# esteinig/sketchy

Hardware: AMD Instinct MI355X
Metric: reads/sec streamed (s=10000,k=16,40k-genome ref) (higher is better)
Workload: dtype u64

## Files before the change

### sketchy_amd/csrc/skx_capi.hip

```cpp
#include <dlfcn.h>
#include <hip/hip_runtime.h>
#include <rccl/rccl.h>

#include <unistd.h>

#include <algorithm>
#include <atomic>
#include <chrono>
#include <cmath>
#include <condition_variable>
#include <cstdarg>
#include <cstdio>
#include <cstdlib>
#include <cstring>
#include <mutex>
#include <string>
#include <thread>
#include <unordered_map>
#include <vector>

#include "sketchy_hip.h"
#include "skx_common.hpp"
#include "skx_genome_groups.hpp"
#include "skx_kernels.hpp"
// ... 965 lines not shown
    u32* h_nq_sink = nullptr;
    u32* h_nd = nullptr;
    u32 *d_rowcnt = nullptr;
    skx::SlotExtents rowcnt_ext;
    bool front_open = false;
    void extents_unknown() { rowcnt_ext.whole(); for (auto& q : ps) { q.smap_ext.whole(); q.mqc_whole = 0xFFu; } }
    u32 *d_gain = nullptr;
    u32 *d_gain_s = nullptr;
    u32 *d_candslot = nullptr;
    u32 *d_candmask = nullptr;
    uint2 *d_lrow = nullptr;
    u32 *d_nlrow = nullptr, *d_gain_l = nullptr, *d_cbase = nullptr, *d_cwl = nullptr, *d_ncwl = nullptr;
    u64 *d_cw = nullptr;
    u64 *d_inb = nullptr, *d_hit = nullptr;
    skx::LongRows long_rows() const { return skx::LongRows{d_lrow, d_nlrow, qcap + 128, d_inb, ref->n_lw}; }
    bool use_pat = false;
    u32 *d_hist = nullptr, *d_nprow = nullptr;
    u64* d_pcw = nullptr;
    u32 npat_pad = 0;
    skx::PatRows pat_rows() const { return skx::PatRows{d_hist, npat_pad, d_gain_l, d_nprow}; }
    skx::RareIndex rare_index() const {
        skx::RareIndex ri = ref->rare_index();
        if (!use_pat) { ri.prec = nullptr; ri.n_pat = 0; }
        if (!static_dense) { ri.qs = nullptr; ri.n_sd = 0; }
        return ri;
    }
    u32 *d_cbad = nullptr, *d_nqc = nullptr;
    u32 *d_spc_g0 = nullptr, *d_spc_grp = nullptr;
    u32 n_pad_c = 0, n_grp_c = 0, cand_seq = 0;
    struct PassSet {
// ... 185 lines not shown
    if (!st) return;
    (void)hipSetDevice(st->device);
    if (st->hs0) (void)hipStreamSynchronize(st->hs0);
    if (st->hs1) (void)hipStreamSynchronize(st->hs1);
    if (st->hs) (void)hipStreamSynchronize(st->hs);
    if (st->hs2) (void)hipStreamSynchronize(st->hs2);
    for (int i = 1; i < skx_stream::kRankLanes; ++i)
        if (st->lane[i].s) (void)hipStreamSynchronize(st->lane[i].s);
    for (int i = 0; i < kSides; ++i) (void)hipFree(st->sd_rows[i]);
    void* ptrs[] = {st->d_bases, st->d_offsets, st->d_pair_h[0], st->d_pair_h[1],
                    st->d_q[0], st->d_q[1], st->d_pair_r[0], st->d_pair_r[1], st->d_pair_q[0], st->d_pair_q[1],
                    st->d_poff_pass[0], st->d_poff_pass[1], st->d_poff_pass[2], st->d_pair_r[2], st->d_nq[0], st->d_nq[1], st->d_win[0], st->d_win[1], st->d_m, st->d_mint, st->d_mq[0], st->d_mq[1],
                    st->d_topk_idx, st->d_topk_sum, st->d_cons, st->d_ev.n_events, st->d_ev.ev_read, st->d_ev.ev_idx, st->d_ev.ev_sum, st->d_ev.ev_codes, st->d_tab_tmp, st->d_rank_idx, st->d_rank_sum, st->d_bsum, st->d_grp_any[0],
                    st->d_grp_any[1], st->d_hbuf, st->d_wb[0], st->d_wb[1], st->d_rowany[0], st->d_rowany[1], st->d_mqext,
                    st->d_qd, st->d_qrow, st->d_sslot, st->d_qinfo, st->d_qloc, st->d_cls_bsum, st->d_nd_hs,
                    st->d_rowcnt, st->d_gain, st->d_gain_s, st->d_candslot, st->d_candmask, st->d_lrow, st->d_nlrow, st->d_gain_l, st->d_cbase, st->d_cwl, st->d_ncwl, st->d_cw, st->d_cbad, st->d_nqc, st->d_spc_g0, st->d_spc_grp, st->d_inb, st->d_hit, st->d_hist, st->d_nprow, st->d_pcw, st->d_ms[0], st->d_ms[1], st->d_mdirty_s};
    for (auto& q : st->ps) {
        for (void* x : {(void*)q.tab, (void*)q.cand, (void*)q.tabc, (void*)q.ncand, (void*)q.mode, (void*)q.any_full, (void*)q.nqc_total, (void*)q.mc, (void*)q.mqc,
                        (void*)q.rowany_c, (void*)q.grp_any_c, (void*)q.smap, (void*)q.pair_qc, (void*)q.nd}) (void)hipFree(x);
        if (q.h_pub) (void)hipHostFree(q.h_pub);
    }
    for (auto& t : st->d_tab) (void)hipFree(t);
    for (int i = 0; i < skx_stream::kRankLanes; ++i) free_lane(st, i);
    for (int i = 1; i < skx_stream::kRankLanes; ++i)
        if (st->own_lane_stream && st->lane[i].s) (void)hipStreamDestroy(st->lane[i].s);
    for (void* p : ptrs) (void)hipFree(p);
    stats_free(st->stats);
    if (st->h_poff) (void)hipHostFree(st->h_poff);
    if (st->h_offsets) (void)hipHostFree(st->h_offsets);
    if (st->h_nq) (void)hipHostFree(st->h_nq);
    if (st->h_nd) (void)hipHostFree(st->h_nd);
// ... 433 lines not shown
            SCHK(hipMalloc(&st->d_cbase, (size_t)nb * (n_pad / 64) * 4));
            SCHK(hipMalloc(&st->d_cwl, (size_t)nb * st->n_pad_c * 4));
            SCHK(hipMalloc(&st->d_ncwl, 64));
            if (ref->d_mlongT) {
                SCHK(hipMalloc(&st->d_inb, (size_t)nb * ref->n_lw * 8));
                SCHK(hipMalloc(&st->d_hit, (size_t)nb * ref->n_lw * 8));
            }
            if (ref->d_prec && ref->n_pat && st->n_grp_c * skx::kRankWords <= skx::pat_words_max()) {
                st->use_pat = true;
                st->npat_pad = (ref->n_pat + 63u) & ~63u;
                SCHK(hipMalloc(&st->d_hist, (size_t)nb * st->npat_pad * 4));
                SCHK(hipMalloc(&st->d_nprow, skx::pass_counter_bytes()));
                SCHK(hipMalloc(&st->d_pcw, (size_t)nb * ref->n_pat * st->n_grp_c * skx::kRankWords * 8));
            }
        }
        SCHK(hipMalloc(&st->d_cbad, 64));
        SCHK(hipMalloc(&st->d_nqc, skx::pass_counter_bytes()));
        std::vector<u32> g0c(n_sp), grpc(st->n_grp_c);
        for (u32 i = 0; i < n_sp; ++i) g0c[i] = i * cap;
        for (u32 i = 0; i < st->n_grp_c; ++i) grpc[i] = i / (cap / (skx::kRankWords * 64));
        SCHK(hipMalloc(&st->d_spc_g0, (size_t)n_sp * 4));
        SCHK(hipMalloc(&st->d_spc_grp, (size_t)st->n_grp_c * 4));
        SCHK(hipMemcpy(st->d_spc_g0, g0c.data(), (size_t)n_sp * 4, hipMemcpyHostToDevice));
        SCHK(hipMemcpy(st->d_spc_grp, grpc.data(), (size_t)st->n_grp_c * 4, hipMemcpyHostToDevice));
        for (auto& q : st->ps) {
            SCHK(hipMalloc(&q.tab, (size_t)(nb + 1) * n_pad * 8));
            SCHK(hipMalloc(&q.cand, (size_t)nb * st->n_pad_c * 4));
            SCHK(hipMalloc(&q.tabc, (size_t)nb * st->n_pad_c * 8));
            SCHK(hipMalloc(&q.ncand, (size_t)nb * n_sp * 4));
            SCHK(hipMalloc(&q.mode, 64)); SCHK(hipMalloc(&q.any_full, 64)); SCHK(hipMalloc(&q.nqc_total, 64));
// ... 103 lines not shown
    const size_t mq_words = (size_t)((n_gw + skx::kRankWords - 1) / skx::kRankWords * skx::kRankWords);
    for (hipStream_t h : {st->hs0, st->hs1, st->hs, st->hs2}) if (h) HIPCHK(hipStreamSynchronize(h));
    for (int i = 1; i < st->n_lanes; ++i) if (st->lane[i].s) HIPCHK(hipStreamSynchronize(st->lane[i].s));
    size_t mem_free = 0, mem_total = 0;
    HIPCHK(hipMemGetInfo(&mem_free, &mem_total));
    const u64 per_row = (st->static_dense ? 0 : (u64)n_pad / 8 * (st->d_mint ? 2 : 1)) + 2 * mq_words * 8 + 2 * (u64)(n_pad / (skx::kRankWords * 64)) / 8 + 1 +
                        5ull * skx::kPassBatchesMax * 4;
    want_rows += st->sd64;
    static const int grow_div = skx::knob("SKX_GROW_DIV") ? std::max(1, atoi(skx::knob("SKX_GROW_DIV"))) : 4;
    u64 rows = std::min<u64>(want_rows, (u64)(mem_free / grow_div) / per_row);
    rows = std::min<u64>(rows, st->pcap) / 64 * 64;
    if (rows <= st->qcap) return SKX_OK;
    u64 *m = nullptr, *mint = nullptr, *mq[2] = {nullptr, nullptr}, *ra[2] = {nullptr, nullptr};
    u32 *wb[2] = {nullptr, nullptr}, *cnt = nullptr, *sm[2] = {nullptr, nullptr};
    uint2* lrow = nullptr;
    auto undo = [&]() { for (void* q : {(void*)m, (void*)mint, (void*)mq[0], (void*)mq[1], (void*)ra[0], (void*)ra[1], (void*)wb[0], (void*)wb[1], (void*)cnt, (void*)sm[0], (void*)sm[1], (void*)lrow}) if (q) (void)hipFree(q); (void)hipGetLastError(); };
    hipError_t e = st->static_dense ? hipSuccess : hipMalloc(&m, (size_t)(rows / 64 + 2) * n_pad * 8);
    if (e == hipSuccess && st->d_mint) e = hipMalloc(&mint, (size_t)(rows / 64 + 2) * n_pad * 8);
    for (int i = 0; i < 2 && e == hipSuccess; ++i) e = hipMalloc(&mq[i], ((size_t)rows + 128) * mq_words * 8);
    for (int i = 0; i < 2 && e == hipSuccess; ++i) e = hipMalloc(&ra[i], (size_t)(n_pad / (skx::kRankWords * 64)) * (rows / 64 + 2) * 8);
    for (int i = 0; i < 2 && e == hipSuccess && st->d_wb[i]; ++i) e = hipMalloc(&wb[i], ((size_t)rows / 64 + 1) * ref->n_tiles * 16);
    if (e == hipSuccess) e = hipMalloc(&cnt, (size_t)skx::kPassBatchesMax * ((size_t)rows + 128) * 4);
    if (e == hipSuccess && st->d_lrow) e = hipMalloc(&lrow, (size_t)skx::kPassBatchesMax * ((size_t)rows + 128) * 8);
    for (int i = 0; i < 2 && e == hipSuccess; ++i) e = hipMalloc(&sm[i], (size_t)skx::kPassBatchesMax * ((size_t)rows + 128) * 4);
    if (e == hipSuccess && m) e = hipMemset(m, 0, (size_t)(rows / 64 + 2) * n_pad * 8);
    for (int i = 0; i < 2 && e == hipSuccess; ++i) e = hipMemset(mq[i], 0, ((size_t)rows + 128) * mq_words * 8);
    for (int i = 0; i < 2 && e == hipSuccess; ++i) e = hipMemset(ra[i], 0, (size_t)(n_pad / (skx::kRankWords * 64)) * (rows / 64 + 2) * 8);
    if (e == hipSuccess) {
        const u32 any[4] = {skx::mq_any_stride(), 0xFFFFFFFFu, skx::mq_any_stride(), 0xFFFFFFFFu};
        e = hipMemcpy(st->d_mqext, any, sizeof(any), hipMemcpyHostToDevice);
    }
    if (e == hipSuccess && mint) e = hipMemset(mint, 0, (size_t)(rows / 64 + 2) * n_pad * 8);
    if (e == hipSuccess) e = hipDeviceSynchronize();
    if (e != hipSuccess) { undo(); return SKX_OK; }
    if (m) { (void)hipFree(st->d_m); st->d_m = m; }
    if (mint) { (void)hipFree(st->d_mint); st->d_mint = mint; }
    for (int i = 0; i < 2; ++i) {
        (void)hipFree(st->d_mq[i]); st->d_mq[i] = mq[i];
        (void)hipFree(st->d_rowany[i]); st->d_rowany[i] = ra[i];
        if (wb[i]) { (void)hipFree(st->d_wb[i]); st->d_wb[i] = wb[i]; }
        (void)hipFree(st->ps[i].smap); st->ps[i].smap = sm[i];
    }
    (void)hipFree(st->d_rowcnt); st->d_rowcnt = cnt;
    st->rowcnt_ext.whole();
    for (auto& q : st->ps) q.smap_ext.whole();
    if (lrow) { (void)hipFree(st->d_lrow); st->d_lrow = lrow; }
    st->qcap = (u32)rows;
    st->mq_stride[0] = st->mq_stride[1] = 0;
    st->qrows_grown += 1;
    return SKX_OK;
}

static int queue_static_scan(skx_stream* st, int b) {
    if (!st->static_dense || st->m_ready[b]) return SKX_OK;
    const skx_ref* ref = st->ref;
    st->m_ready[b] = true;
    if (ref->n_sd == 0) return SKX_OK;
    if (st->reuse_m && st->m_filled[b]) return SKX_OK;
    st->m_filled[b] = true;
    static const bool big_slices = skx::knob("SKX_SCAN_BIGSLICE") && atoi(skx::knob("SKX_SCAN_BIGSLICE")) != 0;
    {
// ... 151 lines not shown
    const bool legacy = update_table && all_ranked && cand_env0 && legacy_env > 0 &&
                        (fresh_overflow || (st->hint_all_overflow && !second_blind && (int)st->legacy_run < legacy_env));
    st->legacy_run = legacy ? st->legacy_run + 1 : 0;
    if (update_table) { st->passes_since_fresh = st->fresh_table ? 1 : st->passes_since_fresh + 1; st->fresh_table = false; }
    const bool long_rows = split_dict && ref->d_mlong != nullptr;
    static const int tail_env = skx::knob("SKX_TAIL_SCALE") ? atoi(skx::knob("SKX_TAIL_SCALE")) : 8;
    const u32 walk_scale = st->tail_pass ? (u32)std::max(1, tail_env) : 1u;
    skx::PassBatches pbt;
    pbt.n = (u32)n_sub;
    for (int i = 0; i < n_sub; ++i) pbt.p_off[i] = subs[i].p_off;
    pbt.p_off[n_sub] = P;
    auto rare_gains = [&](hipStream_t on) -> int {
        const skx::RareIndex ri = st->rare_index();
        const skx::LongRows lrows = st->long_rows();
        const skx::PatRows prows = st->pat_rows();
        skx::launch_gain_sparse(on, d_nd, q_bound, st->d_rowcnt, qstride, (u32)n_sub, n_pad, st->d_gain_s, st->d_sslot, ri, long_rows ? &lrows : nullptr, walk_scale,
                                (long_rows && st->use_pat) ? &prows : nullptr);
        if (long_rows) skx::launch_gain_long(on, lrows, ri, d_nd, st->d_rowcnt, qstride, (u32)n_sub, n_pad, st->d_gain_l, walk_scale);
        if (long_rows && st->use_pat)
            skx::launch_gain_dense(on, ri.pm, nullptr, n_pad, ri.d_npat, ri.n_pat, st->d_hist, st->npat_pad, (u32)n_sub, st->d_gain_l);
        HIPCHK(hipGetLastError());
        return SKX_OK;
    };
    auto row_counts = [&]() -> int {
        skx::launch_pass_hist(hs, d_pair_q, pbt, st->d_rowcnt, qstride);
        return SKX_OK;
    };
    const u32 n_words = nq_rows / 64;
    bool split = false, lean_used = false;
    if (P > 0 && sdm) {
        st->total_passes += 1; st->lean_passes += 1;
        SKXCHK(wait_back());
    } else if (P > 0) {
        static const int split_env = skx::knob("SKX_SCAN_SPLIT") ? atoi(skx::knob("SKX_SCAN_SPLIT")) : -1;
        split = split_env >= 0 ? split_env != 0 : (nd_est * ref->rb / ref->s >= 192);
// ... 82 lines not shown
                    ps.smap_ext.used((u32)n_sub, nq_rows);
                    if (long_rows) {
                        ok = ok && skx::clear_add(pcl, st->d_cw, (size_t)n_sub * n_gw * 8);
                        ok = ok && skx::clear_add(pcl, st->d_cbase, (size_t)n_sub * n_gw * 4, 0xFFu);
                        ok = ok && skx::clear_add(pcl, st->d_ncwl, 64);
                    }
                }
            } else {
                ok = ok && skx::clear_add(pcl, ps.ncand, (size_t)n_sub * n_sp * 4);
            }
            if (!ok) return fail(SKX_ERR_HIP, "internal: the pass's clear table is full or a range is not word-aligned");
            skx::launch_pass_clear(hs, pcl);
        }
        if (P > 0) {
            SKXCHK(row_counts());
            skx::launch_gain_dense(hs, d_m, m_int, n_pad, d_nd, sdm ? ref->n_sd : q_bound, st->d_rowcnt, qstride, (u32)n_sub, st->d_gain,
                                   (sdm && ref->n_species > 1) ? ref->d_segw : nullptr, ref->d_grp_sp);
            if (split_dict) SKXCHK(rare_gains(hs));
        }
        skx::launch_pass_tables(hs, st->d_cum, st->d_gain, (split_dict && P > 0) ? st->d_gain_s : nullptr,
                                (long_rows && P > 0) ? st->d_gain_l : nullptr, (u32)n_sub, n_pad, ps.tab);
        st->d_cum = ps.tab + (size_t)n_sub * n_pad;
        if (ranked) {
            skx::launch_cand_select(hs, ps.tab, n_pad, spc, (u32)n_sub, st->top_k, cap, ps.cand, st->d_candslot, ps.tabc, ps.ncand, st->d_cbad,
                                    st->d_candmask);
            if (fill_mqc) {
                skx::launch_cand_sparse(hs, st->d_sslot, d_nd, q_bound, st->rare_index(), st->d_candmask, st->d_candslot, n_pad, st->d_cbad, (u32)n_sub, st->d_nqc,
                                        ps.smap, qstride, ps.mqc, (size_t)st->n_grp_c * rows_c * skx::kRankWords, rows_c, ps.rowany_c,
                                        st->n_grp_c * (rows_c / 64), ps.grp_any_c, st->n_grp_c, walk_scale);
                if (long_rows) {
                    skx::launch_cand_words(hs, ps.cand, st->n_pad_c, (u32)n_sub, n_gw, st->d_cw, st->d_cbase, st->d_cwl, st->d_ncwl);
                    if (st->d_hit) skx::launch_cand_hit(hs, ps.cand, st->n_pad_c, (u32)n_sub, st->d_cbad, st->rare_index(), st->d_inb, st->d_hit);
// ... 2574 lines not shown
    SKXCHK(flush_pending(st));
    CommWatchdog wd(g_comm_timeout_ms, "ncclAllReduce of the running table", comm->rank, comm->n_ranks, comm->device);
    ncclResult_t r = g_rccl.AllReduce(st->d_cum, st->d_cum, st->ref->n_pad, ncclUint64, ncclSum, comm->comm, st->hs2);
    if (r != ncclSuccess) return fail(SKX_ERR_COMM, "ncclAllReduce: %s", g_rccl.GetErrorString ? g_rccl.GetErrorString(r) : "?");
    HIPCHK(hipStreamSynchronize(st->hs2));
    return SKX_OK;
}
SKX_API void skx_comm_destroy(skx_comm* comm) {
    if (!comm) return;
    if (g_rccl.CommDestroy) (void)g_rccl.CommDestroy(comm->comm);
    delete comm;
}

#ifdef SKX_EXPERIMENTS
namespace skx { void rank_debug_counters(unsigned long long* out, bool reset); }
SKX_API void skx_debug_rank_counters(unsigned long long* out, int reset) { skx::rank_debug_counters(out, reset != 0); }
SKX_API int skx_debug_row_topk(int device, const uint32_t* counts, uint32_t n_rows, uint32_t n, uint32_t top_k, uint32_t bound,
                               uint32_t* top_idx, uint32_t* top_val) {
    if (!counts || !top_idx || !top_val || n_rows < 1 || n < 1) return fail(SKX_ERR_INVALID, "skx_debug_row_topk: bad argument");
    if (top_k < 1 || top_k > SKX_MAX_TOP || top_k > n) return fail(SKX_ERR_INVALID, "skx_debug_row_topk: top_k=%u outside 1..min(n, SKX_MAX_TOP)", top_k);
    SKXCHK(use_device(device));
    const u32 n_pad = (n + kGroupGenomes - 1) / kGroupGenomes * kGroupGenomes;
    DevMem m_cnt, m_sp, m_idx, m_val;
    HIPCHK(m_cnt.need((size_t)n_rows * n_pad * 4));
    HIPCHK(m_sp.need(2 * 4));
    HIPCHK(m_idx.need((size_t)n_rows * top_k * 4));
    HIPCHK(m_val.need((size_t)n_rows * top_k * 4));
    const u32 sp_host[2] = {0u, n};
    HIPCHK(hipMemset(m_cnt.p, 0xFF, (size_t)n_rows * n_pad * 4));
    HIPCHK(hipMemcpy2D(m_cnt.p, (size_t)n_pad * 4, counts, (size_t)n * 4, (size_t)n * 4, n_rows, hipMemcpyHostToDevice));
    HIPCHK(hipMemcpy(m_sp.p, sp_host, sizeof sp_host, hipMemcpyHostToDevice));
// ... 24 lines not shown
```

### sketchy_amd/csrc/skx_kernels.hip

```cpp
#include <algorithm>
#include <cstdlib>
#include <mutex>
#include <type_traits>

#include "skx_common.hpp"
#include "skx_kernels.hpp"

#ifndef SKX_FEW_CANDS
#define SKX_FEW_CANDS 8
#endif
#ifndef SKX_SCAN_ROWS
#define SKX_SCAN_ROWS 8
#endif
#ifndef SKX_SCAN_OCC
#define SKX_SCAN_OCC 1
#endif
#ifndef SKX_SCAN_SPLIT_READS
#define SKX_SCAN_SPLIT_READS 1
#endif
#ifndef SKX_WALK_BLOCKS
#define SKX_WALK_BLOCKS 256
#endif
#ifndef SKX_GAIN_SPARSE_STRIDE
#define SKX_GAIN_SPARSE_STRIDE 16
// ... 3874 lines not shown
        if (m_int) m |= m_int[(size_t)w * n_pad + g];
        if (__ballot(m != 0ull) == 0ull) continue;
        const u32 lo = (u32)m, hi = (u32)(m >> 32);
        const u32 rows = min(64u, nd - w * 64u);
        const u32* c = cnt + (size_t)w * 64u;
        for (u32 j = 0; j < rows; ++j) {
            const u32 bit = j < 32u ? __builtin_amdgcn_ubfe(lo, j, 1u) : __builtin_amdgcn_ubfe(hi, j - 32u, 1u);
#pragma unroll
            for (u32 b = 0; b < NB; ++b) acc[b] += __umul24(bit, c[(size_t)b * row_stride + j]);
        }
    }
#pragma unroll
    for (u32 b = 0; b < NB; ++b)
        if (acc[b]) atomicAdd(&gain[(size_t)b * n_pad + g], acc[b]);
}
__global__ __launch_bounds__(256) void gain_sparse_kernel(const u32* __restrict__ sslot, const u32* __restrict__ n_d, RareIndex ri,
                                                          const u32* __restrict__ cnt, u32 row_stride, u32 n_b, u32 n_pad,
                                                          u32* __restrict__ gain, LongRows lr, PatRows pr) {
    __builtin_amdgcn_s_setprio(2);
    const u32 nd64 = n_d[2], ns = n_d[1], lane = lane_id();
    const u32 wave = blockIdx.x * 4u + (threadIdx.x >> 6), n_waves = gridDim.x * 4u;
    for (u32 r0 = wave * 64u; r0 < ns; r0 += n_waves * 64u) {
        const u32 sr = r0 + lane;
        u32 off = 0, np = 0;
        u32 c[kPassBatchesMax];
        u32 any = 0;
#pragma unroll
        for (u32 b = 0; b < kPassBatchesMax; ++b) c[b] = 0;
        if (sr < ns) {
            const uint2 e = reinterpret_cast<const uint2*>(sslot)[sr];
// ... 73 lines not shown
        }
        u64 longs = __ballot(np > 8u);
        while (longs) {
            const u32 src = (u32)__builtin_ctzll(longs);
            longs &= longs - 1ull;
            const u32 o = __shfl(off, (int)src), n = __shfl(np, (int)src);
            u32 cc[kPassBatchesMax];
#pragma unroll
            for (u32 b = 0; b < kPassBatchesMax; ++b) cc[b] = __shfl(c[b], (int)src);
            for (u32 j = lane; j < n; j += 64u) {
                const u32 g = ri.post[o + j];
#pragma unroll
                for (u32 b = 0; b < kPassBatchesMax; ++b)
                    if (cc[b]) atomicAdd(&gain[((size_t)b * n_pad + g) * kGainSparseStride], cc[b]);
            }
        }
    }
}
__global__ __launch_bounds__(256) void long_rows_kernel(const u32* __restrict__ sslot, const u32* __restrict__ n_d, const u32* __restrict__ cnt,
                                                        u32 row_stride, u32 n_b, LongRows lr) {
    __builtin_amdgcn_s_setprio(3);
    const u32 nd64 = n_d[2], ns = n_d[1], lane = lane_id();
    for (u32 sr0 = (blockIdx.x * 256u + threadIdx.x) & ~63u; sr0 < ns; sr0 += gridDim.x * 256u) {
        const u32 sr = sr0 + lane;
        uint2 e = make_uint2(0u, 0u);
        if (sr < ns) e = reinterpret_cast<const uint2*>(sslot)[sr];
        const bool lng = (e.y & kLongFlag) != 0u;
        if (!__ballot(lng)) continue;
        for (u32 b = 0; b < n_b; ++b) {
            const bool in = lng && cnt[(size_t)b * row_stride + nd64 + sr] != 0u;
            const u64 bal = __ballot(in);
            if (!bal) continue;
            u32 base = 0;
            if (lane == 0u) base = atomicAdd(&lr.nlrow[b * kCtrStride], (u32)__popcll(bal));
            base = (u32)__shfl((int)base, 0);
            if (in) lr.lrow[(size_t)b * lr.lrow_stride + base + (u32)__popcll(bal & lanemask_lt())] = make_uint2(e.x, sr);
        }
    }
}
constexpr u32 kGlPlanes = 23;
__device__ __forceinline__ void planes_add(u64 (&pl)[kGlPlanes], u64 m, u32 k0) {
    u64 carry = m;
#pragma unroll
    for (u32 p = 0; p < kGlPlanes; ++p) {
        if (p >= k0) {
            const u64 t = pl[p] & carry;
            pl[p] ^= carry;
            carry = t;
            if ((p & 3u) == 3u && __ballot(carry != 0ull) == 0ull) return;
        }
    }
// ... 956 lines not shown
    const u32 chunk = std::min(kRareGrpChunk, std::max(1u, (u32)env_int("SKX_RARE_CHUNK", (int)kRareGrpChunk)));
    static const bool sparse_off = env_int("SKX_RARE_SPARSE_WRITES", 1) == 0;
    hipLaunchKernelGGL(rare_to_mq_kernel, dim3(blocks), dim3(256), 0, st, sslot, n_d, ri, mq, nq_rows, n_pad / 64, rowany, grp_any, only_if, chunk,
                       sparse_off ? nullptr : ext);
    if (ext) hipLaunchKernelGGL(mq_extent_kernel, dim3(1), dim3(1), 0, st, ext, nq_rows, n_d, only_if);
}
u32 mq_any_stride() { return kAnyStride; }
void launch_nd_from_nq(hipStream_t st, const u32* n_q, u32* n_d, u32* h_words) {
    hipLaunchKernelGGL(nd_from_nq_kernel, dim3(1), dim3(1), 0, st, n_q, n_d, h_words);
}
void launch_pass_hist(hipStream_t st, const u32* pair_q, const PassBatches& pb, u32* cnt, u32 row_stride) {
    const u32 n = pb.p_off[pb.n];
    if (n == 0) return;
    hipLaunchKernelGGL(pass_hist_kernel, dim3(cdiv(n, 256)), dim3(256), 0, st, pair_q, pb, cnt, row_stride);
}
void launch_gain_dense(hipStream_t st, const u64* m_bits, const u64* m_int, u32 n_pad, const u32* n_d, u32 rows_bound, const u32* cnt, u32 row_stride,
                       u32 n_b, u32* gain, const u32* segw, const u32* grp_sp) {
    const dim3 grid(n_pad / 256, std::max(1u, cdiv(cdiv(rows_bound, 64), kGainWords)));
#define SKX_GAIN(NB) hipLaunchKernelGGL(gain_dense_kernel<NB>, grid, dim3(256), 0, st, m_bits, m_int, n_pad, n_d, cnt, row_stride, gain, segw, grp_sp)
    switch (n_b) {
        case 1: SKX_GAIN(1); break; case 2: SKX_GAIN(2); break; case 3: SKX_GAIN(3); break; case 4: SKX_GAIN(4); break;
        case 5: SKX_GAIN(5); break; case 6: SKX_GAIN(6); break; case 7: SKX_GAIN(7); break; default: SKX_GAIN(8); break;
    }
#undef SKX_GAIN
}
void launch_gain_sparse(hipStream_t st, const u32* n_d, u32 rows_bound, const u32* cnt, u32 row_stride, u32 n_b, u32 n_pad, u32* gain_s,
                        const u32* sslot, const RareIndex& ri, const LongRows* lr, u32 walk_scale, const PatRows* pr) {
    hipLaunchKernelGGL(gain_sparse_kernel, dim3(std::max(1u, std::min(cdiv(rows_bound, 256), kWalkBlocks * std::max(1u, walk_scale)))), dim3(256), 0, st,
                       sslot, n_d, ri, cnt, row_stride, n_b, n_pad, gain_s, lr ? *lr : LongRows{nullptr, nullptr, 0u},
                       (pr && lr && ri.prec) ? *pr : PatRows{nullptr, 0u, nullptr, nullptr});
}
void launch_list_sig(hipStream_t st, const u32* lslot, u32 n_long, const u32* off, const u32* cnt, const u32* post, u32* sig, u64* content) {
// ... 23 lines not shown
    hipLaunchKernelGGL(cand_pat_rows_kernel, dim3(cdiv(ri.n_pat, 4), n_b), dim3(256), 0, st, ri, n_d, candmask, candslot, n_pad, bad, pcw, mqc, mqc_stride,
                       rows_c, rowany_c, rowany_stride, grp_any_c, n_grp_c);
}
void launch_cand_pat_map(hipStream_t st, const LongRows& lr, const PatRows& pr, const RareIndex& ri, const u32* n_d, const u32* candmask,
                         const u32* candslot, u32 n_pad, u32* bad, u32 n_b, u32* nqc, u32* smap, u32 smap_stride, const u64* pcw, u64* mqc,
                         size_t mqc_stride, u32 rows_c, u64* rowany_c, u32 rowany_stride, u32* grp_any_c, u32 n_grp_c, u32 rows_bound, u32 walk_scale) {
    const u32 blocks = std::max(1u, std::min(cdiv(rows_bound, 256), 64u * std::max(1u, walk_scale)));
    hipLaunchKernelGGL(cand_pat_map_kernel, dim3(blocks, n_b), dim3(256), 0, st, lr, pr, ri, n_d, candmask, candslot, n_pad, bad, nqc, smap, smap_stride,
                       pcw, mqc, mqc_stride, rows_c, rowany_c, rowany_stride, grp_any_c, n_grp_c);
}
u32 gain_sparse_stride() { return kGainSparseStride; }
u32 pass_counter_bytes() { return kPassBatchesMax * kCtrStride * 4u; }
void launch_mlong_build(hipStream_t st, const u32* lslot, u32 n_long, const u32* off, const u32* cnt, const u32* post, u64* mlong, u32 n_gw) {
    if (n_long == 0) return;
    hipLaunchKernelGGL(mlong_build_kernel, dim3(cdiv(n_long, 4)), dim3(256), 0, st, lslot, n_long, off, cnt, post, mlong, n_gw);
}
void launch_long_rows(hipStream_t st, const u32* sslot, const u32* n_d, u32 rows_bound, const u32* cnt, u32 row_stride, u32 n_b, const LongRows& lr) {
    hipLaunchKernelGGL(long_rows_kernel, dim3(std::max(1u, std::min(cdiv(rows_bound, 256), (u32)env_int("SKX_G_LONGROWS", 1024)))), dim3(256), 0, st, sslot, n_d, cnt, row_stride, n_b, lr);
}
void launch_gain_long(hipStream_t st, const LongRows& lr, const RareIndex& ri, const u32* n_d, const u32* cnt, u32 row_stride, u32 n_b, u32 n_pad,
                      u32* gain_l, u32 walk_scale) {
    hipLaunchKernelGGL(gain_long_kernel, dim3(cdiv(ri.n_gw, 64), n_b, (u32)env_int("SKX_G_GAINLONG", 8) * std::min(4u, std::max(1u, walk_scale))), dim3(256), 0, st, lr, ri, n_d, cnt, row_stride, n_pad, gain_l);
}
void launch_mlong_transpose(hipStream_t st, const u64* mlong, u32 n_long, u32 n_gw, u64* mlongT, u32 n_lw) {
    if (n_long == 0) return;
    hipLaunchKernelGGL(mlong_transpose_kernel, dim3(n_lw, cdiv(n_gw, 4)), dim3(256), 0, st, mlong, n_long, n_gw, mlongT, n_lw);
}
void launch_cand_hit(hipStream_t st, const u32* cand, u32 n_pad_c, u32 n_b, const u32* bad, const RareIndex& ri, const u64* inb, u64* hit) {
    hipLaunchKernelGGL(cand_hit_kernel, dim3(cdiv(n_pad_c, 4), n_b), dim3(256), 0, st, cand, n_pad_c, bad, ri, inb, hit);
}
void launch_cand_words(hipStream_t st, const u32* cand, u32 n_pad_c, u32 n_b, u32 n_gw, u64* cw, u32* cbase, u32* cwl, u32* ncwl) {
    hipLaunchKernelGGL(cand_words_kernel, dim3(n_b), dim3(1024), 0, st, cand, n_pad_c, n_gw, cw, cbase, cwl, ncwl);
}
// ... 764 lines not shown
```

### sketchy_amd/csrc/skx_kernels.hpp

```cpp
#pragma once
#include <hip/hip_runtime.h>
#include <stddef.h>
#include <stdint.h>

#include <stdlib.h>

#include "skx_pass_clear.hpp"

namespace skx {
typedef unsigned long long u64;
typedef unsigned int u32;

inline const char* knob(const char* name) {
#ifdef SKX_EXPERIMENTS
    return getenv(name);
#else
    (void)name;
    return nullptr;
#endif
}

constexpr int kSketchCap = 2048;
constexpr u32 kSegLen = 64;
constexpr int kRankWords = 8;
// ... 39 lines not shown
                   const u64* mlong = nullptr; const u32* lid = nullptr; const u32* lslot = nullptr; u32 n_gw = 0;
                   const u64* mlongT = nullptr; u32 n_lw = 0;
                   const u32* prec = nullptr; const u32* pat_rep = nullptr; const u64* pm = nullptr; const u32* d_npat = nullptr; u32 n_pat = 0;
                   const u64* qs = nullptr; u32 n_sd = 0; const u32* srow = nullptr; u32 tail0 = 0; };
void launch_collect_dense(hipStream_t st, const u64* key, const u32* off, u64 slots, u64* out, u32* out_slot, u32* n, u32 cap);
void launch_window_seg(hipStream_t st, const u64* lo, const u64* hi, u32 n_bt, u32 n_tiles, const u64* q, const u32* seg, const u32* grp_sp, u32* win);
struct PatRows { u32* hist; u32 hist_stride; u32* gain_x; u32* nprow; };
void launch_list_sig(hipStream_t st, const u32* lslot, u32 n_long, const u32* off, const u32* cnt, const u32* post, u32* sig, u64* content);
void launch_pat_exceptions(hipStream_t st, const u64* mlong, u32 n_gw, u32 n_long, const u32* pat_of, const u32* pat_rep, u32* prec, u32* n_done);
void launch_pat_matrix(hipStream_t st, const u64* mlong, const u32* pat_rep, u32 n_pat, u32 n_gw, u64* pm, u32 n_pad);
u32 pat_record_words();
u32 pat_words_max();
struct LongRows { uint2* lrow; u32* nlrow; u32 lrow_stride; u64* inb = nullptr; u32 n_lw = 0; };
u32 pass_counter_bytes();
void launch_mlong_build(hipStream_t st, const u32* lslot, u32 n_long, const u32* off, const u32* cnt, const u32* post, u64* mlong, u32 n_gw);
void launch_long_rows(hipStream_t st, const u32* sslot, const u32* n_d, u32 rows_bound, const u32* cnt, u32 row_stride, u32 n_b, const LongRows& lr);
void launch_gain_long(hipStream_t st, const LongRows& lr, const RareIndex& ri, const u32* n_d, const u32* cnt, u32 row_stride, u32 n_b, u32 n_pad,
                      u32* gain_l, u32 walk_scale = 1);
void launch_mlong_transpose(hipStream_t st, const u64* mlong, u32 n_long, u32 n_gw, u64* mlongT, u32 n_lw);
void launch_cand_hit(hipStream_t st, const u32* cand, u32 n_pad_c, u32 n_b, const u32* bad, const RareIndex& ri, const u64* inb, u64* hit);
void launch_cand_words(hipStream_t st, const u32* cand, u32 n_pad_c, u32 n_b, u32 n_gw, u64* cw, u32* cbase, u32* cwl, u32* ncwl);
void launch_cand_long(hipStream_t st, const LongRows& lr, const RareIndex& ri, const u32* n_d, const u64* cw, const u32* cbase, const u32* cwl,
                      const u32* ncwl, u32 n_pad_c, u32* bad, u32 n_b, u32* nqc, u32* smap, u32 smap_stride, u64* mqc, size_t mqc_stride,
                      u32 rows_c, u64* rowany_c, u32 rowany_stride, u32* grp_any_c, u32 n_grp_c, u32 walk_scale = 1, const u64* hit = nullptr );
void launch_rare_count(hipStream_t st, const u64* mat, u64 n_elems, u64* key, u32* cnt, u32 mask, u32* overflow,
                       u64* spmask = nullptr , const u32* grp_sp = nullptr, u32 s = 0);
void launch_rare_fill(hipStream_t st, const u64* mat, u64 n_elems, u32 s, const u64* key, const u32* off, u32* cursor, u32* post, u32 mask);
void launch_classify(hipStream_t st, const u64* q, const u32* n_q, u32 q_bound, const RareIndex& ri, u32* qinfo, u32* qloc, u32* bsum,
                     u64* qd, u32* n_d, u32* qrow, u32* sslot, u32* h_words);
void launch_rare_to_mq(hipStream_t st, const u32* sslot, const u32* n_d, const RareIndex& ri, u64* mq, u32 nq_rows, u32 n_pad, u64* rowany,
                       u32* grp_any, u32 rows_bound, const u32* only_if, u32* ext);
u32 mq_any_stride();
void launch_sparse_fill(hipStream_t st, const u32* sslot, const u32* n_d, const RareIndex& ri, u64* m_bits, u32 n_pad, u32* m_dirty,
                        u32 rows_bound, const u32* only_if = nullptr );
void launch_nd_from_nq(hipStream_t st, const u32* n_q, u32* n_d, u32* h_words);

static const u32 kPassBatchesMax = 8;
static const u32 kCandCap = 1024;
static const u32 kCandRows = 131072;
struct PassBatches { u32 n; u32 p_off[kPassBatchesMax + 1]; };
static_assert(kClearSlotsMax == kPassBatchesMax, "one extent per batch slot");
void launch_pass_clear(hipStream_t st, const PassClear& pc);
u32 pass_counter_stride();
void launch_pass_hist(hipStream_t st, const u32* pair_q, const PassBatches& pb, u32* cnt, u32 row_stride);
void launch_gain_dense(hipStream_t st, const u64* m_bits, const u64* m_int , u32 n_pad, const u32* n_d, u32 rows_bound, const u32* cnt,
                       u32 row_stride, u32 n_b, u32* gain, const u32* segw = nullptr ,
                       const u32* grp_sp = nullptr);
void launch_gain_sparse(hipStream_t st, const u32* n_d, u32 rows_bound, const u32* cnt, u32 row_stride, u32 n_b, u32 n_pad, u32* gain_s,
                        const u32* sslot, const RareIndex& ri, const LongRows* lr, u32 walk_scale, const PatRows* pr = nullptr);
void launch_cand_pat_rows(hipStream_t st, const RareIndex& ri, const u32* n_d, const u32* candmask, const u32* candslot, u32 n_pad, u32* bad, u32 n_b,
                          u64* pcw, u64* mqc, size_t mqc_stride, u32 rows_c, u64* rowany_c, u32 rowany_stride, u32* grp_any_c, u32 n_grp_c);
void launch_cand_pat_map(hipStream_t st, const LongRows& lr, const PatRows& pr, const RareIndex& ri, const u32* n_d, const u32* candmask,
                         const u32* candslot, u32 n_pad, u32* bad, u32 n_b, u32* nqc, u32* smap, u32 smap_stride, const u64* pcw, u64* mqc,
                         size_t mqc_stride, u32 rows_c, u64* rowany_c, u32 rowany_stride, u32* grp_any_c, u32 n_grp_c, u32 rows_bound, u32 walk_scale = 1);
u32 gain_sparse_stride();
void launch_pass_tables(hipStream_t st, const u64* prev, const u32* gain, const u32* gain_s , const u32* gain_l , u32 n_b,
                        u32 n_pad, u64* tab);
void launch_cand_select(hipStream_t st, const u64* tab, u32 n_pad, const Species& sp, u32 n_b, u32 top_k, u32 cap, u32* cand, u32* candslot,
                        u64* tabc, u32* ncand, u32* bad, u32* candmask);
void launch_cand_count(hipStream_t st, const u64* t0, const u64* t1, const Species& sp, u32 top_k, u32* h_out, u32 seq);
void launch_cand_gather_m(hipStream_t st, const u64* m_bits, const u64* m_int , u32 n_pad, const u32* n_d, u32 rows_bound, const u32* cand,
                          u32 n_pad_c, const u32* bad, u32 n_b, u64* mc, u32 words_c);
// ... 144 lines not shown
```

Baseline: 157.5 million.

## Compute dense gain with int8 MFMA over packed row counts

Adds a two-kernel path for dense gain. The first kernel packs per-row counts into int8 MFMA B-fragments, split into 7-bit limbs with an optional second limb pass for large counts. The second kernel expands genome bit masks into byte A-fragments and accumulates with mfma_i32_16x16x64_i8, reducing through shared memory instead of per-thread bit loops with atomics. It also removes the unused long_rows kernel and allocates a per-stream operand buffer that grows with the row capacity. Exactness relies on the limb packing and a row bound of 2^22; the extra packing launch and buffer add overhead.

```diff
diff --git a/sketchy_amd/csrc/skx_capi.hip b/sketchy_amd/csrc/skx_capi.hip
--- a/sketchy_amd/csrc/skx_capi.hip
+++ b/sketchy_amd/csrc/skx_capi.hip
@@ -1003,6 +1003,10 @@
     u64 *d_cw = nullptr;
     u64 *d_inb = nullptr, *d_hit = nullptr;
     skx::LongRows long_rows() const { return skx::LongRows{d_lrow, d_nlrow, qcap + 128, d_inb, ref->n_lw}; }
+    void *d_gop = nullptr;
+    u32 *d_gop_pairs = nullptr, gop_words = 0;
+    u32 gop_words_for(u32 rows) const { return std::max(std::max(rows / 64 + 2, (ref->n_sd + 63u) / 64u), npat_pad / 64); }
+    skx::GainOperand gain_operand() const { return skx::GainOperand{d_gop, d_gop_pairs, gop_words}; }
     bool use_pat = false;
     u32 *d_hist = nullptr, *d_nprow = nullptr;
     u64* d_pcw = nullptr;
@@ -1218,7 +1222,7 @@
                     st->d_topk_idx, st->d_topk_sum, st->d_cons, st->d_ev.n_events, st->d_ev.ev_read, st->d_ev.ev_idx, st->d_ev.ev_sum, st->d_ev.ev_codes, st->d_tab_tmp, st->d_rank_idx, st->d_rank_sum, st->d_bsum, st->d_grp_any[0],
                     st->d_grp_any[1], st->d_hbuf, st->d_wb[0], st->d_wb[1], st->d_rowany[0], st->d_rowany[1], st->d_mqext,
                     st->d_qd, st->d_qrow, st->d_sslot, st->d_qinfo, st->d_qloc, st->d_cls_bsum, st->d_nd_hs,
-                    st->d_rowcnt, st->d_gain, st->d_gain_s, st->d_candslot, st->d_candmask, st->d_lrow, st->d_nlrow, st->d_gain_l, st->d_cbase, st->d_cwl, st->d_ncwl, st->d_cw, st->d_cbad, st->d_nqc, st->d_spc_g0, st->d_spc_grp, st->d_inb, st->d_hit, st->d_hist, st->d_nprow, st->d_pcw, st->d_ms[0], st->d_ms[1], st->d_mdirty_s};
+                    st->d_rowcnt, st->d_gain, st->d_gain_s, st->d_candslot, st->d_candmask, st->d_lrow, st->d_gop, st->d_gop_pairs, st->d_nlrow, st->d_gain_l, st->d_cbase, st->d_cwl, st->d_ncwl, st->d_cw, st->d_cbad, st->d_nqc, st->d_spc_g0, st->d_spc_grp, st->d_inb, st->d_hit, st->d_hist, st->d_nprow, st->d_pcw, st->d_ms[0], st->d_ms[1], st->d_mdirty_s};
     for (auto& q : st->ps) {
         for (void* x : {(void*)q.tab, (void*)q.cand, (void*)q.tabc, (void*)q.ncand, (void*)q.mode, (void*)q.any_full, (void*)q.nqc_total, (void*)q.mc, (void*)q.mqc,
                         (void*)q.rowany_c, (void*)q.grp_any_c, (void*)q.smap, (void*)q.pair_qc, (void*)q.nd}) (void)hipFree(x);
@@ -1682,6 +1686,9 @@
                 SCHK(hipMalloc(&st->d_pcw, (size_t)nb * ref->n_pat * st->n_grp_c * skx::kRankWords * 8));
             }
         }
+        st->gop_words = st->gop_words_for(st->qcap);
+        SCHK(hipMalloc(&st->d_gop, skx::gain_operand_bytes(st->gop_words)));
+        SCHK(hipMalloc(&st->d_gop_pairs, (size_t)st->gop_words * 4));
         SCHK(hipMalloc(&st->d_cbad, 64));
         SCHK(hipMalloc(&st->d_nqc, skx::pass_counter_bytes()));
         std::vector<u32> g0c(n_sp), grpc(st->n_grp_c);
@@ -1815,7 +1822,10 @@
     u64 *m = nullptr, *mint = nullptr, *mq[2] = {nullptr, nullptr}, *ra[2] = {nullptr, nullptr};
     u32 *wb[2] = {nullptr, nullptr}, *cnt = nullptr, *sm[2] = {nullptr, nullptr};
     uint2* lrow = nullptr;
-    auto undo = [&]() { for (void* q : {(void*)m, (void*)mint, (void*)mq[0], (void*)mq[1], (void*)ra[0], (void*)ra[1], (void*)wb[0], (void*)wb[1], (void*)cnt, (void*)sm[0], (void*)sm[1], (void*)lrow}) if (q) (void)hipFree(q); (void)hipGetLastError(); };
+    void* gop = nullptr;
+    u32* gop_pairs = nullptr;
+    const u32 gop_words = st->gop_words_for((u32)rows);
+    auto undo = [&]() { for (void* q : {(void*)m, (void*)mint, (void*)mq[0], (void*)mq[1], (void*)ra[0], (void*)ra[1], (void*)wb[0], (void*)wb[1], (void*)cnt, (void*)sm[0], (void*)sm[1], (void*)lrow, gop, (void*)gop_pairs}) if (q) (void)hipFree(q); (void)hipGetLastError(); };
     hipError_t e = st->static_dense ? hipSuccess : hipMalloc(&m, (size_t)(rows / 64 + 2) * n_pad * 8);
     if (e == hipSuccess && st->d_mint) e = hipMalloc(&mint, (size_t)(rows / 64 + 2) * n_pad * 8);
     for (int i = 0; i < 2 && e == hipSuccess; ++i) e = hipMalloc(&mq[i], ((size_t)rows + 128) * mq_words * 8);
@@ -1823,6 +1833,8 @@
     for (int i = 0; i < 2 && e == hipSuccess && st->d_wb[i]; ++i) e = hipMalloc(&wb[i], ((size_t)rows / 64 + 1) * ref->n_tiles * 16);
     if (e == hipSuccess) e = hipMalloc(&cnt, (size_t)skx::kPassBatchesMax * ((size_t)rows + 128) * 4);
     if (e == hipSuccess && st->d_lrow) e = hipMalloc(&lrow, (size_t)skx::kPassBatchesMax * ((size_t)rows + 128) * 8);
+    if (e == hipSuccess && gop_words > st->gop_words) e = hipMalloc(&gop, skx::gain_operand_bytes(gop_words));
+    if (e == hipSuccess && gop_words > st->gop_words) e = hipMalloc(&gop_pairs, (size_t)gop_words * 4);
     for (int i = 0; i < 2 && e == hipSuccess; ++i) e = hipMalloc(&sm[i], (size_t)skx::kPassBatchesMax * ((size_t)rows + 128) * 4);
     if (e == hipSuccess && m) e = hipMemset(m, 0, (size_t)(rows / 64 + 2) * n_pad * 8);
     for (int i = 0; i < 2 && e == hipSuccess; ++i) e = hipMemset(mq[i], 0, ((size_t)rows + 128) * mq_words * 8);
@@ -1846,6 +1858,7 @@
     st->rowcnt_ext.whole();
     for (auto& q : st->ps) q.smap_ext.whole();
     if (lrow) { (void)hipFree(st->d_lrow); st->d_lrow = lrow; }
+    if (gop && gop_pairs) { (void)hipFree(st->d_gop); (void)hipFree(st->d_gop_pairs); st->d_gop = gop; st->d_gop_pairs = gop_pairs; st->gop_words = gop_words; }
     st->qcap = (u32)rows;
     st->mq_stride[0] = st->mq_stride[1] = 0;
     st->qrows_grown += 1;
@@ -2027,11 +2040,12 @@
         const skx::RareIndex ri = st->rare_index();
         const skx::LongRows lrows = st->long_rows();
         const skx::PatRows prows = st->pat_rows();
+        const skx::GainOperand gop = st->gain_operand();
         skx::launch_gain_sparse(on, d_nd, q_bound, st->d_rowcnt, qstride, (u32)n_sub, n_pad, st->d_gain_s, st->d_sslot, ri, long_rows ? &lrows : nullptr, walk_scale,
                                 (long_rows && st->use_pat) ? &prows : nullptr);
         if (long_rows) skx::launch_gain_long(on, lrows, ri, d_nd, st->d_rowcnt, qstride, (u32)n_sub, n_pad, st->d_gain_l, walk_scale);
         if (long_rows && st->use_pat)
-            skx::launch_gain_dense(on, ri.pm, nullptr, n_pad, ri.d_npat, ri.n_pat, st->d_hist, st->npat_pad, (u32)n_sub, st->d_gain_l);
+            skx::launch_gain_dense(on, ri.pm, nullptr, n_pad, ri.d_npat, ri.n_pat, st->d_hist, st->npat_pad, (u32)n_sub, st->d_gain_l, nullptr, nullptr, &gop);
         HIPCHK(hipGetLastError());
         return SKX_OK;
     };
@@ -2144,8 +2158,9 @@
         }
         if (P > 0) {
             SKXCHK(row_counts());
+            const skx::GainOperand gop = st->gain_operand();
             skx::launch_gain_dense(hs, d_m, m_int, n_pad, d_nd, sdm ? ref->n_sd : q_bound, st->d_rowcnt, qstride, (u32)n_sub, st->d_gain,
-                                   (sdm && ref->n_species > 1) ? ref->d_segw : nullptr, ref->d_grp_sp);
+                                   (sdm && ref->n_species > 1) ? ref->d_segw : nullptr, ref->d_grp_sp, &gop);
             if (split_dict) SKXCHK(rare_gains(hs));
         }
         skx::launch_pass_tables(hs, st->d_cum, st->d_gain, (split_dict && P > 0) ? st->d_gain_s : nullptr,
@@ -4750,7 +4765,9 @@
 
 #ifdef SKX_EXPERIMENTS
 namespace skx { void rank_debug_counters(unsigned long long* out, bool reset); }
+namespace skx { void gain_dense_launches(unsigned long long* out, bool reset); }
 SKX_API void skx_debug_rank_counters(unsigned long long* out, int reset) { skx::rank_debug_counters(out, reset != 0); }
+SKX_API void skx_debug_gain_launches(unsigned long long* out, int reset) { skx::gain_dense_launches(out, reset != 0); }
 SKX_API int skx_debug_row_topk(int device, const uint32_t* counts, uint32_t n_rows, uint32_t n, uint32_t top_k, uint32_t bound,
                                uint32_t* top_idx, uint32_t* top_val) {
     if (!counts || !top_idx || !top_val || n_rows < 1 || n < 1) return fail(SKX_ERR_INVALID, "skx_debug_row_topk: bad argument");
diff --git a/sketchy_amd/csrc/skx_kernels.hip b/sketchy_amd/csrc/skx_kernels.hip
--- a/sketchy_amd/csrc/skx_kernels.hip
+++ b/sketchy_amd/csrc/skx_kernels.hip
@@ -1,4 +1,5 @@
 #include <algorithm>
+#include <atomic>
 #include <cstdlib>
 #include <mutex>
 #include <type_traits>
@@ -3912,6 +3913,94 @@
     for (u32 b = 0; b < NB; ++b)
         if (acc[b]) atomicAdd(&gain[(size_t)b * n_pad + g], acc[b]);
 }
+using v4i = __attribute__((ext_vector_type(4))) int;
+constexpr u32 kGopLaneBytes = 16;
+constexpr u32 kGopWordBytes = 64u * kGopLaneBytes;
+__global__ __launch_bounds__(256) void gain_operand_kernel(const u32* __restrict__ n_d, const u32* __restrict__ cnt, u32 row_stride, u32 n_b,
+                                                           v4i* __restrict__ frag, u32* __restrict__ pairs, u32 words_cap) {
+    __builtin_amdgcn_s_setprio(3);
+    const u32 lane = lane_id(), w = blockIdx.x * 4u + (threadIdx.x >> 6);
+    const u32 nd = n_d[0], n_words = min((nd + 63u) >> 6, words_cap);
+    if (w >= n_words) return;
+    const u32 b = lane & 7u, hi = (lane >> 3) & 1u, r0 = w * 64u + (lane >> 4) * 16u;
+    u32 lo4[4], hi4[4], big = 0;
+#pragma unroll
+    for (u32 d = 0; d < 4u; ++d) {
+        lo4[d] = 0; hi4[d] = 0;
+#pragma unroll
+        for (u32 t = 0; t < 4u; ++t) {
+            const u32 r = r0 + d * 4u + t;
+            const u32 c = (b < n_b && r < nd) ? cnt[(size_t)b * row_stride + r] : 0u;
+            big |= c >> 14;
+            lo4[d] |= ((c >> (7u * hi)) & 127u) << (8u * t);
+            hi4[d] |= ((c >> (14u + 7u * hi)) & 127u) << (8u * t);
+        }
+    }
+    const bool two = __ballot(big != 0u) != 0ull;
+    frag[(size_t)w * 64u + lane] = v4i{(int)lo4[0], (int)lo4[1], (int)lo4[2], (int)lo4[3]};
+    if (two) frag[((size_t)words_cap + w) * 64u + lane] = v4i{(int)hi4[0], (int)hi4[1], (int)hi4[2], (int)hi4[3]};
+    if (lane == 0u) pairs[w] = two ? 2u : 1u;
+}
+__device__ __forceinline__ v4i bits16_to_bytes(u32 x) {
+    v4i a;
+    a.x = (int)((((x >> 0) & 0xFu) * 0x00204081u) & 0x01010101u);
+    a.y = (int)((((x >> 4) & 0xFu) * 0x00204081u) & 0x01010101u);
+    a.z = (int)((((x >> 8) & 0xFu) * 0x00204081u) & 0x01010101u);
+    a.w = (int)((((x >> 12) & 0xFu) * 0x00204081u) & 0x01010101u);
+    return a;
+}
+__global__ __launch_bounds__(256) void gain_dense_mfma_kernel(const u64* __restrict__ m_bits, u32 n_pad, const u32* __restrict__ n_d,
+                                                              const v4i* __restrict__ frag, const u32* __restrict__ pairs, u32 words_cap,
+                                                              u32 words_written, u32 n_b, u32* __restrict__ gain, const u32* __restrict__ segw,
+                                                              const u32* __restrict__ grp_sp) {
+    __builtin_amdgcn_s_setprio(2);
+    __shared__ u32 red[4][kPassBatchesMax][64];
+    const u32 lane = lane_id(), wv = threadIdx.x >> 6, g0 = blockIdx.x * 64u;
+    const u32 nd = n_d[0];
+    u32 w0 = 0, w1 = min(min((nd + 63u) >> 6, words_cap), words_written);
+    if (segw) {
+        const u32 sp = grp_sp[blockIdx.x / kRankWords];
+        w0 = max(w0, segw[2u * sp]); w1 = min(w1, segw[2u * sp + 1u]);
+    }
+    if (w0 >= w1) return;
+    const unsigned short* ms = reinterpret_cast<const unsigned short*>(m_bits);
+    const u32 gi = lane & 15u, q = lane >> 4;
+    v4i acc[4], acc2[4];
+#pragma unroll
+    for (u32 f = 0; f < 4u; ++f) { acc[f] = v4i{0, 0, 0, 0}; acc2[f] = v4i{0, 0, 0, 0}; }
+    for (u32 w = w0 + wv; w < w1; w += 4u) {
+        u32 a[4];
+#pragma unroll
+        for (u32 f = 0; f < 4u; ++f) a[f] = ms[((size_t)w * n_pad + g0 + 16u * f + gi) * 4u + q];
+        if (__ballot((a[0] | a[1] | a[2] | a[3]) != 0u) == 0ull) continue;
+        const v4i b0 = frag[(size_t)w * 64u + lane];
+        const u32 np = (u32)__builtin_amdgcn_readfirstlane((int)pairs[w]);
+        v4i A[4];
+#pragma unroll
+        for (u32 f = 0; f < 4u; ++f) A[f] = bits16_to_bytes(a[f]);
+#pragma unroll
+        for (u32 f = 0; f < 4u; ++f) acc[f] = __builtin_amdgcn_mfma_i32_16x16x64_i8(A[f], b0, acc[f], 0, 0, 0);
+        if (np > 1u) {
+            const v4i b1 = frag[((size_t)words_cap + w) * 64u + lane];
+#pragma unroll
+            for (u32 f = 0; f < 4u; ++f) acc2[f] = __builtin_amdgcn_mfma_i32_16x16x64_i8(A[f], b1, acc2[f], 0, 0, 0);
+        }
+    }
+#pragma unroll
+    for (u32 f = 0; f < 4u; ++f)
+#pragma unroll
+        for (u32 r = 0; r < 4u; ++r) {
+            const u32 v = (u32)acc[f][r] + ((u32)acc2[f][r] << 14);
+            const u32 up = (u32)__shfl_down((int)v, 8, 16);
+            if (gi < 8u) red[wv][gi][16u * f + 4u * q + r] = v + 128u * up;
+        }
+    __syncthreads();
+    for (u32 i = threadIdx.x; i < kPassBatchesMax * 64u; i += 256u) {
+        const u32 b = i >> 6, g = i & 63u;
+        const u32 v = red[0][b][g] + red[1][b][g] + red[2][b][g] + red[3][b][g];
+        if (b < n_b && v) gain[(size_t)b * n_pad + g0 + g] += v;
+    }
+}
 __global__ __launch_bounds__(256) void gain_sparse_kernel(const u32* __restrict__ sslot, const u32* __restrict__ n_d, RareIndex ri,
                                                           const u32* __restrict__ cnt, u32 row_stride, u32 n_b, u32 n_pad,
                                                           u32* __restrict__ gain, LongRows lr, PatRows pr) {
@@ -4015,27 +4104,6 @@
                 for (u32 b = 0; b < kPassBatchesMax; ++b)
                     if (cc[b]) atomicAdd(&gain[((size_t)b * n_pad + g) * kGainSparseStride], cc[b]);
             }
-        }
-    }
-}
-__global__ __launch_bounds__(256) void long_rows_kernel(const u32* __restrict__ sslot, const u32* __restrict__ n_d, const u32* __restrict__ cnt,
-                                                        u32 row_stride, u32 n_b, LongRows lr) {
-    __builtin_amdgcn_s_setprio(3);
-    const u32 nd64 = n_d[2], ns = n_d[1], lane = lane_id();
-    for (u32 sr0 = (blockIdx.x * 256u + threadIdx.x) & ~63u; sr0 < ns; sr0 += gridDim.x * 256u) {
-        const u32 sr = sr0 + lane;
-        uint2 e = make_uint2(0u, 0u);
-        if (sr < ns) e = reinterpret_cast<const uint2*>(sslot)[sr];
-        const bool lng = (e.y & kLongFlag) != 0u;
-        if (!__ballot(lng)) continue;
-        for (u32 b = 0; b < n_b; ++b) {
-            const bool in = lng && cnt[(size_t)b * row_stride + nd64 + sr] != 0u;
-            const u64 bal = __ballot(in);
-            if (!bal) continue;
-            u32 base = 0;
-            if (lane == 0u) base = atomicAdd(&lr.nlrow[b * kCtrStride], (u32)__popcll(bal));
-            base = (u32)__shfl((int)base, 0);
-            if (in) lr.lrow[(size_t)b * lr.lrow_stride + base + (u32)__popcll(bal & lanemask_lt())] = make_uint2(e.x, sr);
         }
     }
 }
@@ -5022,8 +5090,37 @@
     if (n == 0) return;
     hipLaunchKernelGGL(pass_hist_kernel, dim3(cdiv(n, 256)), dim3(256), 0, st, pair_q, pb, cnt, row_stride);
 }
+#ifdef SKX_EXPERIMENTS
+static std::atomic<unsigned long long> g_gain_launches[2];
+void gain_dense_launches(unsigned long long* out, bool reset) {
+    for (int i = 0; i < 2; ++i) { out[i] = g_gain_launches[i].load(); if (reset) g_gain_launches[i] = 0; }
+}
+#endif
+bool gain_dense_by_bits() {
+#ifdef SKX_EXPERIMENTS
+    static const int mfma = env_int("SKX_GAIN_MFMA", 1);
+    return mfma == 0;
+#else
+    return false;
+#endif
+}
+size_t gain_operand_bytes(u32 words_cap) { return (size_t)2 * words_cap * kGopWordBytes; }
 void launch_gain_dense(hipStream_t st, const u64* m_bits, const u64* m_int, u32 n_pad, const u32* n_d, u32 rows_bound, const u32* cnt, u32 row_stride,
-                       u32 n_b, u32* gain, const u32* segw, const u32* grp_sp) {
+                       u32 n_b, u32* gain, const u32* segw, const u32* grp_sp, const GainOperand* op) {
+    if (op && op->frag && !m_int && !gain_dense_by_bits() && n_b <= kPassBatchesMax && cdiv(rows_bound, 64) <= op->words_cap && rows_bound <= (1u << 22)) {
+        const u32 words = std::max(1u, cdiv(rows_bound, 64));
+#ifdef SKX_EXPERIMENTS
+        g_gain_launches[0] += 1;
+#endif
+        hipLaunchKernelGGL(gain_operand_kernel, dim3(cdiv(words, 4)), dim3(256), 0, st, n_d, cnt, row_stride, n_b, reinterpret_cast<v4i*>(op->frag), op->pairs,
+                           op->words_cap);
+        hipLaunchKernelGGL(gain_dense_mfma_kernel, dim3(n_pad / 64), dim3(256), 0, st, m_bits, n_pad, n_d, reinterpret_cast<const v4i*>(op->frag), op->pairs,
+                           op->words_cap, words, n_b, gain, segw, grp_sp);
+        return;
+    }
+#ifdef SKX_EXPERIMENTS
+    g_gain_launches[1] += 1;
+#endif
     const dim3 grid(n_pad / 256, std::max(1u, cdiv(cdiv(rows_bound, 64), kGainWords)));
 #define SKX_GAIN(NB) hipLaunchKernelGGL(gain_dense_kernel<NB>, grid, dim3(256), 0, st, m_bits, m_int, n_pad, n_d, cnt, row_stride, gain, segw, grp_sp)
     switch (n_b) {
@@ -5077,9 +5174,6 @@
 void launch_mlong_build(hipStream_t st, const u32* lslot, u32 n_long, const u32* off, const u32* cnt, const u32* post, u64* mlong, u32 n_gw) {
     if (n_long == 0) return;
     hipLaunchKernelGGL(mlong_build_kernel, dim3(cdiv(n_long, 4)), dim3(256), 0, st, lslot, n_long, off, cnt, post, mlong, n_gw);
-}
-void launch_long_rows(hipStream_t st, const u32* sslot, const u32* n_d, u32 rows_bound, const u32* cnt, u32 row_stride, u32 n_b, const LongRows& lr) {
-    hipLaunchKernelGGL(long_rows_kernel, dim3(std::max(1u, std::min(cdiv(rows_bound, 256), (u32)env_int("SKX_G_LONGROWS", 1024)))), dim3(256), 0, st, sslot, n_d, cnt, row_stride, n_b, lr);
 }
 void launch_gain_long(hipStream_t st, const LongRows& lr, const RareIndex& ri, const u32* n_d, const u32* cnt, u32 row_stride, u32 n_b, u32 n_pad,
                       u32* gain_l, u32 walk_scale) {
diff --git a/sketchy_amd/csrc/skx_kernels.hpp b/sketchy_amd/csrc/skx_kernels.hpp
--- a/sketchy_amd/csrc/skx_kernels.hpp
+++ b/sketchy_amd/csrc/skx_kernels.hpp
@@ -77,7 +77,6 @@
 struct LongRows { uint2* lrow; u32* nlrow; u32 lrow_stride; u64* inb = nullptr; u32 n_lw = 0; };
 u32 pass_counter_bytes();
 void launch_mlong_build(hipStream_t st, const u32* lslot, u32 n_long, const u32* off, const u32* cnt, const u32* post, u64* mlong, u32 n_gw);
-void launch_long_rows(hipStream_t st, const u32* sslot, const u32* n_d, u32 rows_bound, const u32* cnt, u32 row_stride, u32 n_b, const LongRows& lr);
 void launch_gain_long(hipStream_t st, const LongRows& lr, const RareIndex& ri, const u32* n_d, const u32* cnt, u32 row_stride, u32 n_b, u32 n_pad,
                       u32* gain_l, u32 walk_scale = 1);
 void launch_mlong_transpose(hipStream_t st, const u64* mlong, u32 n_long, u32 n_gw, u64* mlongT, u32 n_lw);
@@ -106,9 +105,12 @@
 void launch_pass_clear(hipStream_t st, const PassClear& pc);
 u32 pass_counter_stride();
 void launch_pass_hist(hipStream_t st, const u32* pair_q, const PassBatches& pb, u32* cnt, u32 row_stride);
+struct GainOperand { void* frag; u32* pairs; u32 words_cap; };
+size_t gain_operand_bytes(u32 words_cap);
+bool gain_dense_by_bits();
 void launch_gain_dense(hipStream_t st, const u64* m_bits, const u64* m_int , u32 n_pad, const u32* n_d, u32 rows_bound, const u32* cnt,
                        u32 row_stride, u32 n_b, u32* gain, const u32* segw = nullptr ,
-                       const u32* grp_sp = nullptr);
+                       const u32* grp_sp = nullptr, const GainOperand* op = nullptr);
 void launch_gain_sparse(hipStream_t st, const u32* n_d, u32 rows_bound, const u32* cnt, u32 row_stride, u32 n_b, u32 n_pad, u32* gain_s,
                         const u32* sslot, const RareIndex& ri, const LongRows* lr, u32 walk_scale, const PatRows* pr = nullptr);
 void launch_cand_pat_rows(hipStream_t st, const RareIndex& ri, const u32* n_d, const u32* candmask, const u32* candslot, u32 n_pad, u32* bad, u32 n_b,
```

After: 165.3 million (median of 6 runs). 5.0% higher.
